# bjack205/LQR.jl

Hardware: NVIDIA B200
Metric: batched LQR KKT solves/sec (FP64) (higher is better)
Workload: dtype f64

## Files before the change

lqr.jl_b200/csrc/api.cu:

```cuda
#include <cstdio>
#include <cstring>

#include "common.cuh"

int32_t lqrb_fail(lqrb_context *h, int32_t code, const std::string &msg) {
    if (h) h->err = msg;
    return code;
}

int32_t lqrb_cuda_fail(lqrb_context *h, cudaError_t e, const char *what) {
    if (h) h->err = std::string(what) + ": " + cudaGetErrorString(e);
    return 1000 + (int32_t)e;
}

void *lqrb_scratch(lqrb_context *h, int slot, size_t bytes, int lane) {
    if (bytes == 0) bytes = 16;
    void *&cur = h->scratch[slot][lane];
    size_t &have = h->scratch_bytes[slot][lane];
    if (have >= bytes) return cur;
    if (cur) {
        cudaDeviceSynchronize();
        cudaFree(cur);
        cur = nullptr;
        have = 0;
    }
    void *p = nullptr;
    cudaError_t e = cudaMalloc(&p, bytes);
    if (e != cudaSuccess) {
        lqrb_cuda_fail(h, e, "cudaMalloc(scratch)");
        return nullptr;
    }
    cur = p;
    have = bytes;
    return p;
}

void *lqrb_pinned(lqrb_context *h, int lane, size_t bytes) {
    if (bytes == 0) bytes = 16;
    if (h->pinned_bytes[lane] >= bytes) return h->pinned[lane];
    if (h->pinned[lane]) {
        cudaStreamSynchronize(h->stream);
        cudaFreeHost(h->pinned[lane]);
        h->pinned[lane] = nullptr;
        h->pinned_bytes[lane] = 0;
    }
    void *p = nullptr;
    cudaError_t e = cudaMallocHost(&p, bytes);
    if (e != cudaSuccess) {
        lqrb_cuda_fail(h, e, "cudaMallocHost");
        return nullptr;
    }
    h->pinned[lane] = p;
    h->pinned_bytes[lane] = bytes;
    return p;
}

extern "C" int32_t lqrb_version(void) { return LQRB_VERSION; }

extern "C" int32_t lqrb_device_count(int32_t *count) {
    if (!count) return -1;
    int c = 0;
    cudaError_t e = cudaGetDeviceCount(&c);
    if (e != cudaSuccess) {
        cudaGetLastError();
        *count = 0;
        return 1000 + (int32_t)e;
    }
    *count = c;
    return 0;
}

extern "C" int32_t lqrb_create(lqrb_handle_t *handle, int32_t device) {
    if (!handle) return -1;
    *handle = nullptr;
    int c = 0;
    cudaError_t e = cudaGetDeviceCount(&c);
    if (e != cudaSuccess) {
        cudaGetLastError();
        return 1000 + (int32_t)e;
    }
    if (device < 0 || device >= c) return -2;
    lqrb_context *h = new lqrb_context();
    h->device = device;
    if ((e = cudaSetDevice(device)) != cudaSuccess) {
        delete h;
        return 1000 + (int32_t)e;
    }
    cudaDeviceProp prop;
    if ((e = cudaGetDeviceProperties(&prop, device)) != cudaSuccess) {
        delete h;
        return 1000 + (int32_t)e;
    }
    if (prop.major != 10) {
        delete h;
        return -2;
    }
    h->sm_count = prop.multiProcessorCount;
    cudaStreamCreateWithFlags(&h->own_stream, cudaStreamNonBlocking);
    cudaStreamCreateWithFlags(&h->copy_stream[0], cudaStreamNonBlocking);
    cudaStreamCreateWithFlags(&h->copy_stream[1], cudaStreamNonBlocking);
    for (auto &ev : h->ev) cudaEventCreateWithFlags(&ev, cudaEventDisableTiming);
    h->stream = h->own_stream;
    *handle = h;
    return 0;
}

extern "C" int32_t lqrb_destroy(lqrb_handle_t h) {
    if (!h) return -1;
    cudaSetDevice(h->device);
    cudaDeviceSynchronize();
    for (auto &slot : h->scratch)
        for (void *p : slot)
            if (p) cudaFree(p);
    for (void *p : h->pinned)
        if (p) cudaFreeHost(p);
    for (auto &kv : h->maps)
        if (kv.second.dev) cudaFree((void *)kv.second.dev);
    for (auto &kv : h->blobs)
        if (kv.second) cudaFree(kv.second);
    for (auto &ev : h->ev)
        if (ev) cudaEventDestroy(ev);
    cudaStreamDestroy(h->own_stream);
    cudaStreamDestroy(h->copy_stream[0]);
    cudaStreamDestroy(h->copy_stream[1]);
    delete h;
    return 0;
}

extern "C" const char *lqrb_last_error_string(lqrb_handle_t h) {
    return h ? h->err.c_str() : "null handle";
}

extern "C" int32_t lqrb_set_stream(lqrb_handle_t h, void *s) {
    if (!h) return -1;
    h->stream = s ? (cudaStream_t)s : h->own_stream;
    return 0;
}

extern "C" int32_t lqrb_synchronize(lqrb_handle_t h) {
    if (!h) return -1;
    LQRB_CUDA(h, cudaSetDevice(h->device));
    LQRB_CUDA(h, cudaStreamSynchronize(h->stream));
    return 0;
}

extern "C" int64_t lqrb_launch_count(lqrb_handle_t h) { return h ? h->launches : -1; }

extern "C" const char *lqrb_last_kernel_name(lqrb_handle_t h) {
    return h ? h->kernel_name.c_str() : "";
}

extern "C" int32_t lqrb_set_option(lqrb_handle_t h, const char *name, int64_t value) {
    if (!h) return -1;
    if (!name) return -2;
    h->options[name] = value;
    return 0;
}

extern "C" int64_t lqrb_padded_batch(int64_t batch) { return round_up(batch, LQRB_TILE); }

extern "C" int64_t lqrb_num_vars(int32_t n, int32_t m, int32_t N) {
    return (int64_t)N * n + (int64_t)(N - 1) * m;
}

extern "C" int64_t lqrb_num_cons(int32_t n, int32_t N, const int32_t *p) {
    int64_t P = (int64_t)(N - 1) * n;
    if (p)
        for (int k = 0; k < N; ++k) P += p[k];
    return P;
}

extern "C" int32_t lqrb_riccati_layout(int32_t n, int32_t m, int32_t N, int32_t flags,
                                       lqrb_riccati_layout_t *out) {
    if (n < 1) return -1;
    if (m < 1) return -2;
    if (N < 2) return -3;
    if (!out) return -5;
    out->rows_per_knot = lqrb_riccati_knot_rows(n, m);
    out->knot_count = (flags & LQRB_FLAG_LTI) ? 1 : N - 1;
    out->term_rows = tri(n) + 2 * n;
// ... 174 lines not shown
```

lqr.jl_b200/csrc/common.cuh:

```cuda
#pragma once
#include <cuda_runtime.h>
#include <stdint.h>

#include <algorithm>
#include <functional>
#include <map>
#include <string>
#include <vector>

#include "../../include/lqrb200.h"

#define LQRB_TILE 32

__host__ __device__ __forceinline__ int64_t packed_index(int64_t rows, int tile_w, int64_t row,
                                                         int64_t inst) {
    return ((inst / tile_w) * rows + row) * tile_w + (inst % tile_w);
}

__host__ __device__ constexpr int tri(int k) { return k * (k + 1) / 2; }
__host__ __device__ constexpr int tri_idx(int i, int j) { return j * (j + 1) / 2 + i; }
__host__ __device__ constexpr int sym_idx(int i, int j) { return i <= j ? tri_idx(i, j) : tri_idx(j, i); }

__host__ __device__ constexpr int hess_rows(int n, int mk, int hess) {
    return hess == LQRB_HESS_DIAG ? n + mk : hess == LQRB_HESS_BLOCKDIAG ? tri(n) + tri(mk) : tri(n + mk);
}

enum ScratchSlot {
    SCR_GAINS = 0,
    SCR_FACT,
    SCR_STAGE_A,
    SCR_STAGE_B,
    SCR_PACK_IN,
    SCR_PACK_IN2,
    SCR_PACK_OUT,
    SCR_PACK_OUT2,
    SCR_PACK_OUT3,
    SCR_MISC,
    SCR_SQP0,
    SCR_SQP1,
    SCR_SQP2,
    SCR_SQP3,
    SCR_KEEP_DATA,
    SCR_KEEP_REC,
    SCR_REFINE,
    SCR_REFINE_LIST,
    SCR_RICCATI_PAD,
    SCR_COUNT
};

struct Lane {
    cudaStream_t stream;
    int index;
};

struct RowMap;
struct DevMap {
    const RowMap *dev = nullptr;
    int64_t rows = 0;
};

struct lqrb_context {
    int device = 0;
    int sm_count = 148;
    cudaStream_t stream = nullptr;
    cudaStream_t own_stream = nullptr;
    cudaStream_t copy_stream[2] = {nullptr, nullptr};
    cudaEvent_t ev[8] = {};
    std::string err;
    std::string kernel_name;
    int64_t launches = 0;
    void *scratch[SCR_COUNT][2] = {};
    size_t scratch_bytes[SCR_COUNT][2] = {};
    void *pinned[2] = {};
    size_t pinned_bytes[2] = {};
    std::map<std::string, int64_t> options;
    std::map<std::string, struct DevMap> maps;
    std::map<std::string, void *> blobs;
    std::vector<int32_t> last_cond;
    int64_t last_refined = 0;
    std::string kept_key;
    int64_t kept_batch = 0;

    int64_t opt(const char *name, int64_t dflt) const {
        auto it = options.find(name);
        return it == options.end() ? dflt : it->second;
    }
};

int32_t lqrb_fail(lqrb_context *h, int32_t code, const std::string &msg);
int32_t lqrb_cuda_fail(lqrb_context *h, cudaError_t e, const char *what);
void *lqrb_scratch(lqrb_context *h, int slot, size_t bytes, int lane = 0);
void *lqrb_pinned(lqrb_context *h, int lane, size_t bytes);

struct HostArray {
    const void *ptr;
    int64_t bytes;
};
using ChunkBody = std::function<int32_t(Lane lane, int64_t cb, const void *const *in, void *const *out)>;
int32_t lqrb_for_chunks(lqrb_context *h, int64_t batch, int64_t chunk, const std::vector<HostArray> &inputs,
                        const std::vector<HostArray> &outputs, const ChunkBody &body);

#define LQRB_CUDA(h, call)                                              \
    do {                                                                \
        cudaError_t e__ = (call);                                       \
        if (e__ != cudaSuccess) return lqrb_cuda_fail((h), e__, #call); \
    } while (0)

#define LQRB_LAUNCH_CHECK(h, name)                                                    \
    do {                                                                              \
        (h)->launches++;                                                              \
        cudaError_t e__ = cudaGetLastError();                                         \
        if (e__ != cudaSuccess) return lqrb_cuda_fail((h), e__, "launch of " name);   \
    } while (0)

static inline int64_t round_up(int64_t a, int64_t b) { return (a + b - 1) / b * b; }

__host__ __device__ constexpr int lqrb_riccati_knot_rows(int n, int m) {
    const int f = n * n + n * m + n * (n + 1) / 2 + m * (m + 1) / 2 + n + m;
    return ((n == 8 || n == 12) && m <= 4) ? ((f + 1) & ~1) : f;
}

struct RowMap {
    int32_t array;
    int32_t offset;
    double fill;
};
#define LQRB_MAX_ARRAYS 16
struct ArrayTable {
    const double *ptr[LQRB_MAX_ARRAYS];
    int64_t stride[LQRB_MAX_ARRAYS];
};
struct ArrayTableOut {
    double *ptr[LQRB_MAX_ARRAYS];
    int64_t stride[LQRB_MAX_ARRAYS];
};

DevMap lqrb_get_map(lqrb_context *h, const std::string &key, std::vector<RowMap> (*build)(const int *),
                    const int *args);
DevMap lqrb_get_map(lqrb_context *h, const std::string &key, const std::vector<RowMap> &map);
DevMap lqrb_identity_map(lqrb_context *h, int64_t rows);
int32_t lqrb_gather_pack(lqrb_context *h, const DevMap &map, const ArrayTable &src, int64_t batch,
                         int tile_w, double *packed, cudaStream_t s);
int32_t lqrb_scatter_unpack(lqrb_context *h, const DevMap &map, const ArrayTableOut &dst,
                            int64_t batch, int tile_w, const double *packed, cudaStream_t s);

int lqrb_riccati_tile(const lqrb_context *h, int n, int m);
// ... 7 lines not shown
```

lqr.jl_b200/csrc/riccati.cu:

```cuda
#include <algorithm>
#include <cstdio>

#include "riccati_kernels.cuh"
#include "riccati_dmma_kernels.cuh"
#include "riccati_cta_kernels.cuh"

#define RICCATI_SIZES(X)                                                                                              \
    X(Tpi, 2, 1) X(Tpi, 3, 2) X(Tpi, 4, 1) X(Tpi, 4, 2) X(Tpi, 6, 3) X(Tpi, 2, 2) X(Tpi, 3, 1) X(Tpi, 3, 3)           \
    X(Tpi, 4, 3) X(Tpi, 5, 1) X(Tpi, 5, 2) X(Tpi, 5, 3) X(Tpi, 6, 1) X(Tpi, 6, 2)                                     \
    X(Dmma, 8, 1) X(Dmma, 8, 2) X(Dmma, 8, 3) X(Dmma, 8, 4) X(Dmma, 12, 1) X(Dmma, 12, 2) X(Dmma, 12, 3)              \
    X(Dmma, 12, 4)                                                                                                    \
    X(Cta, 16, 8) X(Cta, 16, 16) X(Cta, 24, 8) X(Cta, 24, 16) X(Cta, 32, 8) X(Cta, 32, 16) X(Cta, 48, 16) X(Cta, 64, 16)

namespace {
enum class RiccatiFamily { Tpi, Dmma, Cta, Pad, Coop };
struct RiccatiRoute {
    RiccatiFamily family;
    int n2 = 0, m2 = 0;
};
}

static RiccatiRoute riccati_route(const lqrb_context *h, int n, int m, bool data_aligned) {
    if (h->opt("riccati_variant", 0) == 2) return {RiccatiFamily::Coop};
    RiccatiFamily own = RiccatiFamily::Coop;
#define X(F_, N_, M_) \
    if (n == N_ && m == M_) own = RiccatiFamily::F_;
    RICCATI_SIZES(X)
#undef X
    if (own == RiccatiFamily::Tpi || (data_aligned && own != RiccatiFamily::Coop)) return {own};
    if (data_aligned && h->opt("riccati_pad", 1) != 0) {
#define X(F_, N_, M_) \
    if (RiccatiFamily::F_ != RiccatiFamily::Tpi && n <= N_ && m <= M_) return {RiccatiFamily::Pad, N_, M_};
        RICCATI_SIZES(X)
#undef X
    }
    return {RiccatiFamily::Coop};
}

int lqrb_riccati_tile(const lqrb_context *h, int n, int m) {
    return riccati_route(h, n, m, true).family == RiccatiFamily::Tpi ? LQRB_TILE : 1;
}

static std::vector<RowMap> riccati_knot_map(int n, int m, int N, int flags) {
    const int Kn = (flags & LQRB_FLAG_LTI) ? 1 : N - 1;
    std::vector<RowMap> map;
    map.reserve((size_t)Kn * (n * n + n * m + tri(n) + tri(m) + n + m));
    for (int k = 0; k < Kn; ++k) {
        for (int e = 0; e < n * n; ++e) map.push_back({0, k * n * n + e, 0.0});
        for (int e = 0; e < n * m; ++e) map.push_back({1, k * n * m + e, 0.0});
        for (int j = 0; j < n; ++j)
            for (int i = 0; i <= j; ++i) map.push_back({2, k * n * n + i + j * n, 0.0});
        for (int j = 0; j < m; ++j)
            for (int i = 0; i <= j; ++i) map.push_back({3, k * m * m + i + j * m, 0.0});
        for (int e = 0; e < n; ++e) map.push_back({4, k * n + e, 0.0});
        for (int e = 0; e < m; ++e) map.push_back({5, k * m + e, 0.0});
        if (lqrb_riccati_knot_rows(n, m) > n * n + n * m + tri(n) + tri(m) + n + m) map.push_back({-1, 0, 0.0});
    }
    return map;
}

static std::vector<RowMap> riccati_term_map(int n) {
    std::vector<RowMap> map;
    for (int j = 0; j < n; ++j)
        for (int i = 0; i <= j; ++i) map.push_back({6, i + j * n, 0.0});
    for (int e = 0; e < n; ++e) map.push_back({7, e, 0.0});
    for (int e = 0; e < n; ++e) map.push_back({8, e, 0.0});
    return map;
}

static std::vector<RowMap> riccati_gain_map(int n, int m, int N) {
    std::vector<RowMap> map;
    for (int k = 0; k < N - 1; ++k) {
        for (int e = 0; e < m * n; ++e) map.push_back({0, k * m * n + e, 0.0});
        for (int e = 0; e < m; ++e) map.push_back({1, k * m + e, 0.0});
    }
    return map;
}

static std::string key(const char *tag, int a, int b, int c, int d) {
    char buf[96];
    snprintf(buf, sizeof buf, "%s:%d:%d:%d:%d", tag, a, b, c, d);
    return buf;
}

static int32_t check_dims(lqrb_context *h, int n, int m, int N, int64_t batch) {
    if (!h) return -1;
    if (n < 1 || n > 128) return lqrb_fail(h, -2, "n out of range [1,128]");
    if (m < 1 || m > n) return lqrb_fail(h, -3, "m out of range [1,n]");
    if (N < 2) return lqrb_fail(h, -4, "N must be >= 2");
    if (batch < 0) return lqrb_fail(h, -5, "batch must be >= 0");
    return 0;
}

template <int n, int m>
static int32_t launch_tpi(lqrb_context *h, int N, int64_t batch, int lti, const double *knots,
                          const double *term, double *Z, double *gains, int32_t *info,
                          cudaStream_t s) {
    constexpr bool SMALL = (n * n + n * m) <= 20;
    constexpr int THREADS = SMALL ? 64 : 128, MINB = SMALL ? 8 : 1;
    const unsigned grid = (unsigned)((batch + THREADS - 1) / THREADS);
    if (lti) riccati_tpi_kernel<n, m, true, THREADS, MINB><<<grid, THREADS, 0, s>>>(knots, term, Z, gains, info, N, batch);
    else riccati_tpi_kernel<n, m, false, THREADS, MINB><<<grid, THREADS, 0, s>>>(knots, term, Z, gains, info, N, batch);
    char nm[64];
    snprintf(nm, sizeof nm, "riccati_tpi<%d,%d>%s%s", n, m, lti ? "[lti]" : "", SMALL ? "[64x8]" : "[128x1]");
    h->kernel_name = nm;
    LQRB_LAUNCH_CHECK(h, "riccati_tpi_kernel");
    return 0;
}

static int32_t launch_coop(lqrb_context *h, int n, int m, int N, int64_t batch, int lti,
                           const double *knots, const double *term, double *Z, double *gains,
                           int32_t *info, cudaStream_t s) {
    const size_t per = riccati_coop_smem_doubles(n, m) * sizeof(double);
    char nm[64];
    if (n + m <= 24) {
        constexpr int G = 32, THREADS = 128;
        const size_t smem = per * (THREADS / G);
        auto kern = riccati_coop_kernel<G, THREADS>;
        LQRB_CUDA(h, cudaFuncSetAttribute(kern, cudaFuncAttributeMaxDynamicSharedMemorySize, (int)smem));
        const unsigned grid = (unsigned)((batch + THREADS / G - 1) / (THREADS / G));
        kern<<<grid, THREADS, smem, s>>>(knots, term, Z, gains, info, n, m, N, lti, batch);
        snprintf(nm, sizeof nm, "riccati_coop<G=32>(n=%d,m=%d)", n, m);
    } else {
        constexpr int G = 256, THREADS = 256;
        if (per > 227 * 1024) return lqrb_fail(h, -2, "n,m too large for the shared-memory Riccati kernel");
        auto kern = riccati_coop_kernel<G, THREADS>;
        LQRB_CUDA(h, cudaFuncSetAttribute(kern, cudaFuncAttributeMaxDynamicSharedMemorySize, (int)per));
        kern<<<(unsigned)batch, THREADS, per, s>>>(knots, term, Z, gains, info, n, m, N, lti, batch);
        snprintf(nm, sizeof nm, "riccati_coop<G=256>(n=%d,m=%d)", n, m);
    }
    h->kernel_name = nm;
    LQRB_LAUNCH_CHECK(h, "riccati_coop_kernel");
    return 0;
}

template <int n, int m>
static int32_t launch_dmma(lqrb_context *h, int N, int64_t batch, int lti, const double *knots,
                           const double *term, double *Z, double *gains, int32_t *info,
                           cudaStream_t s) {
    constexpr int STAGES = 3, WARPS = 4, MINB = m == 1 ? 6 : 5;
    const size_t smem = rdmma::riccati_dmma_warp_smem(rdmma::Map<n, m>::F, STAGES) * WARPS;
    auto kern = rdmma::riccati_dmma_kernel<n, m, STAGES, WARPS, MINB>;
    LQRB_CUDA(h, cudaFuncSetAttribute(kern, cudaFuncAttributeMaxDynamicSharedMemorySize, (int)smem));
    const unsigned grid = (unsigned)((batch + WARPS - 1) / WARPS);
    kern<<<grid, WARPS * 32, smem, s>>>(knots, term, Z, gains, info, N, lti, batch);
    char nm[64];
    snprintf(nm, sizeof nm, "riccati_dmma<%d,%d>%s", n, m, lti ? "[lti]" : "");
    h->kernel_name = nm;
    LQRB_LAUNCH_CHECK(h, "riccati_dmma_kernel");
    return 0;
}

template <int n, int m>
static int32_t launch_cta(lqrb_context *h, int N, int64_t batch, int lti, const double *knots,
                          const double *term, double *Z, double *gains, int32_t *info, cudaStream_t s) {
    using C = rcta::Cfg<n, m>;
    auto kern = rcta::riccati_cta_kernel<n, m>;
    LQRB_CUDA(h, cudaFuncSetAttribute(kern, cudaFuncAttributeMaxDynamicSharedMemorySize, (int)C::SMEM));
    kern<<<(unsigned)batch, C::THREADS, C::SMEM, s>>>(knots, term, Z, gains, info, N, lti, batch);
    char nm[64];
    snprintf(nm, sizeof nm, "riccati_cta_dmma<%d,%d>%s", n, m, lti ? "[lti]" : "");
    h->kernel_name = nm;
    LQRB_LAUNCH_CHECK(h, "riccati_cta_kernel");
    return 0;
}

template <RiccatiFamily F, int n, int m>
static int32_t launch_sized(lqrb_context *h, int N, int64_t batch, int lti, const double *knots, const double *term,
                            double *Z, double *gains, int32_t *info, cudaStream_t s) {
    if constexpr (F == RiccatiFamily::Tpi) return launch_tpi<n, m>(h, N, batch, lti, knots, term, Z, gains, info, s);
    else if constexpr (F == RiccatiFamily::Dmma) return launch_dmma<n, m>(h, N, batch, lti, knots, term, Z, gains, info, s);
    else return launch_cta<n, m>(h, N, batch, lti, knots, term, Z, gains, info, s);
}

static int32_t launch_tuned(lqrb_context *h, RiccatiFamily family, int n, int m, int N, int64_t batch, int lti,
                            const double *knots, const double *term, double *Z, double *gains, int32_t *info,
                            cudaStream_t s) {
#define X(F_, N_, M_)                                                     \
    if (family == RiccatiFamily::F_ && n == N_ && m == M_)                \
        return launch_sized<RiccatiFamily::F_, N_, M_>(h, N, batch, lti, knots, term, Z, gains, info, s);
    RICCATI_SIZES(X)
#undef X
    return lqrb_fail(h, 1, "no tuned Riccati kernel for this size");
}


namespace {
struct RiccatiPadMaps {
    std::vector<RowMap> knots, term, z, gains;
};
}

static RiccatiPadMaps riccati_pad_maps(int n, int m, int N, int Kn, int n2, int m2) {
    RiccatiPadMaps M;
    const int F = lqrb_riccati_knot_rows(n, m), F2 = lqrb_riccati_knot_rows(n2, m2);
    const int nn = n * n, nm = n * m, tn = tri(n), tm = tri(m);
    for (int k = 0; k < Kn; ++k) {
        const int32_t b = k * F;
        const size_t start = M.knots.size();
        for (int j = 0; j < n2; ++j)
            for (int i = 0; i < n2; ++i) M.knots.push_back((i < n && j < n) ? RowMap{0, b + i + j * n, 0.0} : RowMap{-1, 0, 0.0});
        for (int j = 0; j < m2; ++j)
            for (int i = 0; i < n2; ++i)
                M.knots.push_back((i < n && j < m) ? RowMap{0, b + nn + i + j * n, 0.0} : RowMap{-1, 0, 0.0});
        for (int j = 0; j < n2; ++j)
            for (int i = 0; i <= j; ++i)
                M.knots.push_back(j < n ? RowMap{0, b + nn + nm + j * (j + 1) / 2 + i, 0.0} : RowMap{-1, 0, i == j ? 1.0 : 0.0});
        for (int j = 0; j < m2; ++j)
            for (int i = 0; i <= j; ++i)
                M.knots.push_back(j < m ? RowMap{0, b + nn + nm + tn + j * (j + 1) / 2 + i, 0.0} : RowMap{-1, 0, i == j ? 1.0 : 0.0});
        for (int i = 0; i < n2; ++i) M.knots.push_back(i < n ? RowMap{0, b + nn + nm + tn + tm + i, 0.0} : RowMap{-1, 0, 0.0});
        for (int i = 0; i < m2; ++i) M.knots.push_back(i < m ? RowMap{0, b + nn + nm + tn + tm + n + i, 0.0} : RowMap{-1, 0, 0.0});
        while (M.knots.size() - start < (size_t)F2) M.knots.push_back(RowMap{-1, 0, 0.0});
    }
    for (int j = 0; j < n2; ++j)
        for (int i = 0; i <= j; ++i) M.term.push_back(j < n ? RowMap{0, j * (j + 1) / 2 + i, 0.0} : RowMap{-1, 0, i == j ? 1.0 : 0.0});
    for (int i = 0; i < n2; ++i) M.term.push_back(i < n ? RowMap{0, tn + i, 0.0} : RowMap{-1, 0, 0.0});
    for (int i = 0; i < n2; ++i) M.term.push_back(i < n ? RowMap{0, tn + n + i, 0.0} : RowMap{-1, 0, 0.0});
    for (int k = 0; k < N; ++k) {
        for (int i = 0; i < n2; ++i) M.z.push_back(i < n ? RowMap{0, k * (n + m) + i, 0.0} : RowMap{-1, 0, 0.0});
        if (k < N - 1)
            for (int i = 0; i < m2; ++i) M.z.push_back(i < m ? RowMap{0, k * (n + m) + n + i, 0.0} : RowMap{-1, 0, 0.0});
    }
    const int GR = m * n + m;
    for (int k = 0; k < N - 1; ++k) {
        for (int j = 0; j < n2; ++j)
            for (int c = 0; c < m2; ++c) M.gains.push_back((c < m && j < n) ? RowMap{0, k * GR + c + m * j, 0.0} : RowMap{-1, 0, 0.0});
        for (int c = 0; c < m2; ++c) M.gains.push_back(c < m ? RowMap{0, k * GR + m * n + c, 0.0} : RowMap{-1, 0, 0.0});
    }
    return M;
}

static int32_t riccati_solve_padded(lqrb_context *h, int n, int m, int N, int n2, int m2, int64_t batch, int flags,
                                    const double *knots, const double *term, double *Z, double *gains, int32_t *info,
                                    Lane lane) {
    const RiccatiFamily family = riccati_route(h, n2, m2, true).family;
    if (family != RiccatiFamily::Dmma && family != RiccatiFamily::Cta)
        return lqrb_fail(h, 1, "padded Riccati size has no tensor-core kernel");
    const int lti = (flags & LQRB_FLAG_LTI) ? 1 : 0;
    const int Kn = lti ? 1 : N - 1;
    const int64_t F = lqrb_riccati_knot_rows(n, m), F2 = lqrb_riccati_knot_rows(n2, m2);
    const int64_t TR = tri(n) + 2 * n, TR2 = tri(n2) + 2 * n2;
    const int64_t ZR = (int64_t)N * n + (int64_t)(N - 1) * m, ZR2 = (int64_t)N * n2 + (int64_t)(N - 1) * m2;
    const int64_t GR = (int64_t)(N - 1) * (m * n + m), GR2 = (int64_t)(N - 1) * (m2 * n2 + m2);
    const std::string k0 = key("rpad", n, m, N, Kn) + key("->", n2, m2, 0, 0);
    DevMap mk, mt, mz, mg;
    if (h->maps.find(k0 + ":g") == h->maps.end()) {
        const RiccatiPadMaps M = riccati_pad_maps(n, m, N, Kn, n2, m2);
        mk = lqrb_get_map(h, k0 + ":k", M.knots);
        mt = lqrb_get_map(h, k0 + ":t", M.term);
        mz = lqrb_get_map(h, k0 + ":z", M.z);
        mg = lqrb_get_map(h, k0 + ":g", M.gains);
    } else {
        mk = h->maps[k0 + ":k"];
        mt = h->maps[k0 + ":t"];
        mz = h->maps[k0 + ":z"];
        mg = h->maps[k0 + ":g"];
    }
    if (mk.rows != Kn * F2 || mt.rows != TR2 || mz.rows != ZR2 || mg.rows != GR2) return lqrb_fail(h, 1, "pad map size mismatch");
    const int64_t per = Kn * F2 + TR2 + ZR2 + GR2;
    int64_t chunk = std::max<int64_t>(LQRB_TILE, ((int64_t)2 << 30) / (per * 8) / LQRB_TILE * LQRB_TILE);
    chunk = std::min(chunk, lqrb_padded_batch(batch));
    const size_t slice = ((size_t)chunk * per * 8 + 255) / 256 * 256;
    char *base = (char *)lqrb_scratch(h, SCR_RICCATI_PAD, slice, lane.index);
    if (!base) return 1000 + (int)cudaErrorMemoryAllocation;
    double *knots2 = (double *)base, *term2 = knots2 + chunk * Kn * F2, *Z2 = term2 + chunk * TR2, *gains2 = Z2 + chunk * ZR2;
    std::string name;
    for (int64_t first = 0; first < batch; first += chunk) {
        const int64_t cb = std::min(chunk, batch - first);
        ArrayTable src = {};
        src.ptr[0] = knots + first * Kn * F;
        src.stride[0] = Kn * F;
        int32_t rc = lqrb_gather_pack(h, mk, src, cb, 1, knots2, lane.stream);
        if (rc) return rc;
        src.ptr[0] = term + first * TR;
        src.stride[0] = TR;
        rc = lqrb_gather_pack(h, mt, src, cb, 1, term2, lane.stream);
        if (rc) return rc;
        rc = launch_tuned(h, family, n2, m2, N, cb, lti, knots2, term2, Z2, gains2, info ? info + first : nullptr,
                          lane.stream);
        if (rc) return rc;
        name = h->kernel_name;
        ArrayTableOut o = {};
        o.ptr[0] = Z + first * ZR;
        o.stride[0] = ZR;
        rc = lqrb_scatter_unpack(h, mz, o, cb, 1, Z2, lane.stream);
        if (rc) return rc;
        o.ptr[0] = gains + first * GR;
        o.stride[0] = GR;
        rc = lqrb_scatter_unpack(h, mg, o, cb, 1, gains2, lane.stream);
        if (rc) return rc;
    }
    char nm[64];
    snprintf(nm, sizeof nm, " <- (%d,%d) padded", n, m);
    h->kernel_name = name + nm;
    return 0;
}

static int32_t riccati_solve_on(lqrb_context *h, int n, int m, int N, int64_t batch, int flags,
                                const double *knots, const double *term, double *Z, double *gains,
                                int32_t *info, Lane lane) {
    if (batch == 0) return 0;
    const RiccatiRoute r = riccati_route(h, n, m, ((uintptr_t)knots & 15) == 0);
    const int lti = (flags & LQRB_FLAG_LTI) ? 1 : 0;
    switch (r.family) {
    case RiccatiFamily::Pad:
        return riccati_solve_padded(h, n, m, N, r.n2, r.m2, batch, flags, knots, term, Z, gains, info, lane);
    case RiccatiFamily::Tpi:
    case RiccatiFamily::Dmma:
    case RiccatiFamily::Cta:
        return launch_tuned(h, r.family, n, m, N, batch, lti, knots, term, Z, gains, info, lane.stream);
    case RiccatiFamily::Coop:
        break;
    }
    return launch_coop(h, n, m, N, batch, lti, knots, term, Z, gains, info, lane.stream);
}

extern "C" int32_t lqrb_riccati_solve_packed_f64(lqrb_handle_t h, int32_t n, int32_t m, int32_t N,
                                                 int64_t batch, int32_t flags, const double *knots,
                                                 const double *term, double *Z, double *gains,
                                                 int32_t *info) {
    int32_t rc = check_dims(h, n, m, N, batch);
    if (rc) return rc;
    if (!knots) return lqrb_fail(h, -7, "knots is NULL");
    if (!term) return lqrb_fail(h, -8, "term is NULL");
    if (!Z) return lqrb_fail(h, -9, "Z is NULL");
    LQRB_CUDA(h, cudaSetDevice(h->device));
    if (!gains) {
        const size_t bytes = (size_t)lqrb_padded_batch(batch) * (N - 1) * (m * n + m) * sizeof(double);
        gains = (double *)lqrb_scratch(h, SCR_GAINS, bytes);
        if (!gains) return 1000 + (int)cudaErrorMemoryAllocation;
    }
    return riccati_solve_on(h, n, m, N, batch, flags, knots, term, Z, gains, info, Lane{h->stream, 0});
}

static int32_t riccati_pack_on(lqrb_context *h, int n, int m, int N, int64_t batch, int flags,
                               const double *A, const double *B, const double *Q, const double *R,
                               const double *q, const double *r, const double *Qf, const double *qf,
                               const double *x0, double *knots, double *term, cudaStream_t s) {
    const int Kn = (flags & LQRB_FLAG_LTI) ? 1 : N - 1;
    const int tile = lqrb_riccati_tile(h, n, m);
    ArrayTable t = {};
    const double *ptrs[9] = {A, B, Q, R, q, r, Qf, qf, x0};
    const int64_t strides[9] = {(int64_t)Kn * n * n, (int64_t)Kn * n * m, (int64_t)Kn * n * n,
                                (int64_t)Kn * m * m, (int64_t)Kn * n,     (int64_t)Kn * m,
                                (int64_t)n * n,      n,                   n};
    for (int i = 0; i < 9; ++i) {
        t.ptr[i] = ptrs[i];
        t.stride[i] = strides[i];
    }
    DevMap km = lqrb_get_map(h, key("rk", n, m, N, flags & LQRB_FLAG_LTI), riccati_knot_map(n, m, N, flags));
    DevMap tm = lqrb_get_map(h, key("rt", n, 0, 0, 0), riccati_term_map(n));
    int32_t rc = lqrb_gather_pack(h, km, t, batch, tile, knots, s);
    if (rc) return rc;
    return lqrb_gather_pack(h, tm, t, batch, tile, term, s);
}

extern "C" int32_t lqrb_riccati_pack_f64(lqrb_handle_t h, int32_t n, int32_t m, int32_t N,
                                         int64_t batch, int32_t flags, const double *A,
                                         const double *B, const double *Q, const double *R,
                                         const double *q, const double *r, const double *Qf,
                                         const double *qf, const double *x0, double *knots,
                                         double *term) {
    int32_t rc = check_dims(h, n, m, N, batch);
    if (rc) return rc;
    if (!A) return lqrb_fail(h, -7, "A is NULL");
    if (!B) return lqrb_fail(h, -8, "B is NULL");
    if (!Q) return lqrb_fail(h, -9, "Q is NULL");
    if (!R) return lqrb_fail(h, -10, "R is NULL");
    if (!Qf) return lqrb_fail(h, -13, "Qf is NULL");
    if (!x0) return lqrb_fail(h, -15, "x0 is NULL");
    if (!knots) return lqrb_fail(h, -16, "knots is NULL");
    if (!term) return lqrb_fail(h, -17, "term is NULL");
    LQRB_CUDA(h, cudaSetDevice(h->device));
    return riccati_pack_on(h, n, m, N, batch, flags, A, B, Q, R, q, r, Qf, qf, x0, knots, term, h->stream);
}

static int32_t riccati_unpack_on(lqrb_context *h, int n, int m, int N, int64_t batch,
                                 const double *Zp, const double *gains, double *Z, double *K,
                                 double *kff, cudaStream_t s) {
    const int tile = lqrb_riccati_tile(h, n, m);
    const int64_t NN = lqrb_num_vars(n, m, N);
    ArrayTableOut t = {};
    t.ptr[0] = Z;
    t.stride[0] = NN;
    int32_t rc = lqrb_scatter_unpack(h, lqrb_identity_map(h, NN), t, batch, tile, Zp, s);
    if (rc) return rc;
    if (K || kff) {
// ... 161 lines not shown
```

lqr.jl_b200/csrc/riccati_kernels.cuh:

```cuda
#pragma once
#include "smallmat.cuh"

template <int n, int m>
struct RiccatiRows {
    static constexpr int oA = 0, oB = n * n, oQ = oB + n * m, oR = oQ + tri(n), oq = oR + tri(m),
                         orr = oq + n, F = lqrb_riccati_knot_rows(n, m);
    static constexpr int TR = tri(n) + 2 * n;
    static constexpr int GR = m * n + m;
    static constexpr int W = n + m;
};

template <int n, int m>
__device__ __forceinline__ int riccati_step(const double *A, const double *B, const double *Q,
                                            const double *R, const double *q, const double *r,
                                            double *P, double *p, double *K, double *kff) {
    double PB[n * m], PA[n * n], E[tri(m)], Einv[m], Kraw[m * n], rr[m];
    SM_UNROLL
    for (int j = 0; j < m; ++j)
        SM_UNROLL
        for (int i = 0; i < n; ++i) {
            double s = 0.0;
            SM_UNROLL
            for (int l = 0; l < n; ++l) s = fma(P[sym_idx(i, l)], B[l + j * n], s);
            PB[i + j * n] = s;
        }
    SM_UNROLL
    for (int j = 0; j < n; ++j)
        SM_UNROLL
        for (int i = 0; i < n; ++i) {
            double s = 0.0;
            SM_UNROLL
            for (int l = 0; l < n; ++l) s = fma(P[sym_idx(i, l)], A[l + j * n], s);
            PA[i + j * n] = s;
        }
    SM_UNROLL
    for (int j = 0; j < m; ++j)
        SM_UNROLL
        for (int i = 0; i <= j; ++i) {
            double s = R[tri_idx(i, j)];
            SM_UNROLL
            for (int l = 0; l < n; ++l) s = fma(B[l + i * n], PB[l + j * n], s);
            E[tri_idx(i, j)] = s;
        }
    SM_UNROLL
    for (int j = 0; j < n; ++j)
        SM_UNROLL
        for (int i = 0; i < m; ++i) {
            double s = 0.0;
            SM_UNROLL
            for (int l = 0; l < n; ++l) s = fma(B[l + i * n], PA[l + j * n], s);
            Kraw[i + j * m] = s;
            K[i + j * m] = s;
        }
    SM_UNROLL
    for (int i = 0; i < m; ++i) {
        double s = r[i];
        SM_UNROLL
        for (int l = 0; l < n; ++l) s = fma(B[l + i * n], p[l], s);
        rr[i] = s;
        kff[i] = s;
    }
    const int st = chol_packed<m>(E, Einv);
    SM_UNROLL
    for (int j = 0; j < n; ++j) solve_chol<m>(E, Einv, K + j * m);
    solve_chol<m>(E, Einv, kff);
    double pn[n];
    SM_UNROLL
    for (int i = 0; i < n; ++i) {
        double s = q[i];
        SM_UNROLL
        for (int l = 0; l < n; ++l) s = fma(A[l + i * n], p[l], s);
        SM_UNROLL
        for (int l = 0; l < m; ++l) s = fma(-K[l + i * m], rr[l], s);
        pn[i] = s;
    }
    SM_UNROLL
    for (int j = 0; j < n; ++j)
        SM_UNROLL
        for (int i = 0; i <= j; ++i) {
            double s = Q[tri_idx(i, j)];
            SM_UNROLL
            for (int l = 0; l < n; ++l) s = fma(A[l + i * n], PA[l + j * n], s);
            SM_UNROLL
            for (int l = 0; l < m; ++l) s = fma(-Kraw[l + i * m], K[l + j * m], s);
            P[tri_idx(i, j)] = s;
        }
    SM_UNROLL
    for (int i = 0; i < n; ++i) p[i] = pn[i];
    return st;
}

template <int n, int m, bool LTI, int THREADS, int MINB>
__global__ void __launch_bounds__(THREADS, MINB)
    riccati_tpi_kernel(const double *__restrict__ knots, const double *__restrict__ term,
                       double *__restrict__ Z, double *__restrict__ gains,
                       int32_t *__restrict__ info, int N, int64_t batch) {
    using L = RiccatiRows<n, m>;
    const int64_t inst = (int64_t)blockIdx.x * THREADS + threadIdx.x;
    if (inst >= batch) return;
    const int64_t tile = inst >> 5;
    const int lane = (int)(inst & 31);
    const int Kn = LTI ? 1 : N - 1;
    const double *kb = knots + tile * Kn * L::F * 32 + lane;
    const double *tb = term + tile * L::TR * 32 + lane;
    double *zb = Z + tile * ((int64_t)N * n + (int64_t)(N - 1) * m) * 32 + lane;
    double *gb = gains + tile * (int64_t)(N - 1) * L::GR * 32 + lane;

    double P[tri(n)], p[n];
    SM_UNROLL
    for (int e = 0; e < tri(n); ++e) P[e] = ld_stream(tb + e * 32);
    SM_UNROLL
    for (int e = 0; e < n; ++e) p[e] = ld_stream(tb + (tri(n) + e) * 32);

    double A[n * n], B[n * m];
    int st_all = 0;
    for (int k = N - 2; k >= 0; --k) {
        const double *kp = kb + (int64_t)(LTI ? 0 : k) * L::F * 32;
        double Q[tri(n)], R[tri(m)], q[n], r[m];
        SM_UNROLL
        for (int e = 0; e < n * n; ++e) A[e] = ld_keep(kp + (L::oA + e) * 32);
        SM_UNROLL
        for (int e = 0; e < n * m; ++e) B[e] = ld_keep(kp + (L::oB + e) * 32);
        SM_UNROLL
        for (int e = 0; e < tri(n); ++e) Q[e] = ld_stream(kp + (L::oQ + e) * 32);
        SM_UNROLL
        for (int e = 0; e < tri(m); ++e) R[e] = ld_stream(kp + (L::oR + e) * 32);
        SM_UNROLL
        for (int e = 0; e < n; ++e) q[e] = ld_stream(kp + (L::oq + e) * 32);
        SM_UNROLL
        for (int e = 0; e < m; ++e) r[e] = ld_stream(kp + (L::orr + e) * 32);
        double K[m * n], kff[m];
        const int st = riccati_step<n, m>(A, B, Q, R, q, r, P, p, K, kff);
        if (st != 0 && st_all == 0) st_all = (k + 1) * 1000 + st;
        double *gk = gb + (int64_t)k * L::GR * 32;
        SM_UNROLL
        for (int e = 0; e < m * n; ++e) gk[e * 32] = K[e];
        SM_UNROLL
        for (int e = 0; e < m; ++e) gk[(m * n + e) * 32] = kff[e];
    }
    if (info) info[inst] = st_all;

    double x[n];
    SM_UNROLL
    for (int e = 0; e < n; ++e) x[e] = ld_stream(tb + (tri(n) + n + e) * 32);
    for (int k = 0; k < N - 1; ++k) {
        const double *kp = kb + (int64_t)(LTI ? 0 : k) * L::F * 32;
        const double *gk = gb + (int64_t)k * L::GR * 32;
        double K[m * n], kff[m], u[m], xn[n];
        SM_UNROLL
        for (int e = 0; e < n * n; ++e) A[e] = ld_stream(kp + (L::oA + e) * 32);
        SM_UNROLL
        for (int e = 0; e < n * m; ++e) B[e] = ld_stream(kp + (L::oB + e) * 32);
        SM_UNROLL
        for (int e = 0; e < m * n; ++e) K[e] = gk[e * 32];
        SM_UNROLL
        for (int e = 0; e < m; ++e) kff[e] = gk[(m * n + e) * 32];
        double *zk = zb + (int64_t)k * L::W * 32;
        SM_UNROLL
        for (int i = 0; i < n; ++i) __stcs(zk + i * 32, x[i]);
        SM_UNROLL
        for (int i = 0; i < m; ++i) {
            double s = -kff[i];
            SM_UNROLL
            for (int l = 0; l < n; ++l) s = fma(-K[i + l * m], x[l], s);
            u[i] = s;
            __stcs(zk + (n + i) * 32, s);
        }
        SM_UNROLL
        for (int i = 0; i < n; ++i) {
            double s = 0.0;
            SM_UNROLL
            for (int l = 0; l < n; ++l) s = fma(A[i + l * n], x[l], s);
            SM_UNROLL
            for (int l = 0; l < m; ++l) s = fma(B[i + l * n], u[l], s);
            xn[i] = s;
        }
        SM_UNROLL
        for (int i = 0; i < n; ++i) x[i] = xn[i];
    }
    double *zN = zb + (int64_t)(N - 1) * L::W * 32;
    SM_UNROLL
    for (int i = 0; i < n; ++i) __stcs(zN + i * 32, x[i]);
}

template <int G>
__device__ __forceinline__ void group_sync() {
    if (G <= 32)
        __syncwarp();
    else
        __syncthreads();
}

__host__ __device__ inline size_t riccati_coop_smem_doubles(int n, int m) {
    return (size_t)4 * n * n + 4 * n * m + m * m + 4 * n + 3 * m + 8;
}

template <int G, int THREADS>
__global__ void __launch_bounds__(THREADS)
    riccati_coop_kernel(const double *__restrict__ knots, const double *__restrict__ term,
                        double *__restrict__ Z, double *__restrict__ gains,
                        int32_t *__restrict__ info, int n, int m, int N, int lti, int64_t batch) {
    extern __shared__ double smem[];
    constexpr int IPC = THREADS / G;
    const int g = threadIdx.x / G, t = threadIdx.x % G;
    const int64_t inst_raw = (int64_t)blockIdx.x * IPC + g;
    const bool active = inst_raw < batch;
    const int64_t inst = active ? inst_raw : batch - 1;
    const int nn = n * n, nm = n * m, tn = tri(n), tm = tri(m);
    const int F = lqrb_riccati_knot_rows(n, m), TR = tn + 2 * n, GR = m * n + m, W = n + m;
    const int Kn = lti ? 1 : N - 1;
    double *s = smem + (size_t)g * riccati_coop_smem_doubles(n, m);
    double *P = s, *Pn = P + nn, *PA = Pn + nn, *A = PA + nn, *B = A + nn, *PB = B + nm,
           *Kraw = PB + nm, *K = Kraw + nm, *E = K + nm, *p = E + m * m, *pn = p + n, *x = pn + n,
           *xn = x + n, *rr = xn + n, *kff = rr + m, *u = kff + m;
    const double *rec = knots + inst * (int64_t)Kn * F;
    const double *tb = term + inst * TR;
    double *zb = Z + inst * ((int64_t)N * n + (int64_t)(N - 1) * m);
    double *gb = gains + inst * (int64_t)(N - 1) * GR;
    int st_all = 0;

    for (int e = t; e < nn; e += G) {
        const int i = e % n, j = e / n;
        P[e] = tb[sym_idx(i, j)];
    }
    for (int e = t; e < n; e += G) p[e] = tb[tn + e];
    group_sync<G>();

    for (int k = N - 2; k >= 0; --k) {
        const double *kp = rec + (int64_t)(lti ? 0 : k) * F;
        const double *Qp = kp + nn + nm, *Rp = Qp + tn, *qp = Rp + tm, *rp = qp + n;
        for (int e = t; e < nn; e += G) A[e] = kp[e];
        for (int e = t; e < nm; e += G) B[e] = kp[nn + e];
        group_sync<G>();
        for (int e = t; e < nn + nm; e += G) {
            const bool isA = e < nn;
            const int ee = isA ? e : e - nn;
            const int i = ee % n, j = ee / n;
            const double *col = (isA ? A : B) + j * n;
            double acc = 0.0;
// ... 116 lines not shown
```

Before: 116.7 million.

## Pin late-knot dynamics and gains in L2 with evict_last hints across passes

In the time-varying Riccati kernel, the A/B loads and the K/kff gain stores for the first W knots, which the forward pass reads first, now use an L2 evict_last cache policy. W is sized from a fraction of the device L2 capacity divided by the per-knot footprint across the batch. After the forward pass uses a knot, its lines are demoted back to evict_normal with applypriority. The goal is to turn the forward pass's DRAM reads of A, B and the gains into L2 hits, at the cost of extra applypriority instructions and possible L2 contention with other traffic.

```diff
diff --git a/lqr.jl_b200/csrc/api.cu b/lqr.jl_b200/csrc/api.cu
--- a/lqr.jl_b200/csrc/api.cu
+++ b/lqr.jl_b200/csrc/api.cu
@@ -96,6 +96,7 @@
         return -2;
     }
     h->sm_count = prop.multiProcessorCount;
+    h->l2_bytes = prop.l2CacheSize;
     cudaStreamCreateWithFlags(&h->own_stream, cudaStreamNonBlocking);
     cudaStreamCreateWithFlags(&h->copy_stream[0], cudaStreamNonBlocking);
     cudaStreamCreateWithFlags(&h->copy_stream[1], cudaStreamNonBlocking);
diff --git a/lqr.jl_b200/csrc/common.cuh b/lqr.jl_b200/csrc/common.cuh
--- a/lqr.jl_b200/csrc/common.cuh
+++ b/lqr.jl_b200/csrc/common.cuh
@@ -62,6 +62,7 @@
 struct lqrb_context {
     int device = 0;
     int sm_count = 148;
+    int64_t l2_bytes = 126 << 20;
     cudaStream_t stream = nullptr;
     cudaStream_t own_stream = nullptr;
     cudaStream_t copy_stream[2] = {nullptr, nullptr};
diff --git a/lqr.jl_b200/csrc/riccati.cu b/lqr.jl_b200/csrc/riccati.cu
--- a/lqr.jl_b200/csrc/riccati.cu
+++ b/lqr.jl_b200/csrc/riccati.cu
@@ -92,6 +92,11 @@
     return 0;
 }
 
+#ifndef RTPI_SHARE
+#define RTPI_SHARE 0.5
+#endif
+constexpr double RTPI_L2_SHARE = RTPI_SHARE;
+
 template <int n, int m>
 static int32_t launch_tpi(lqrb_context *h, int N, int64_t batch, int lti, const double *knots,
                           const double *term, double *Z, double *gains, int32_t *info,
@@ -99,8 +104,10 @@
     constexpr bool SMALL = (n * n + n * m) <= 20;
     constexpr int THREADS = SMALL ? 64 : 128, MINB = SMALL ? 8 : 1;
     const unsigned grid = (unsigned)((batch + THREADS - 1) / THREADS);
-    if (lti) riccati_tpi_kernel<n, m, true, THREADS, MINB><<<grid, THREADS, 0, s>>>(knots, term, Z, gains, info, N, batch);
-    else riccati_tpi_kernel<n, m, false, THREADS, MINB><<<grid, THREADS, 0, s>>>(knots, term, Z, gains, info, N, batch);
+    const int64_t kept_per_knot = lqrb_padded_batch(batch) * (n * n + n * m + m * n + m) * 8;
+    const int W = (int)std::min<int64_t>(N - 1, (int64_t)(RTPI_L2_SHARE * h->l2_bytes) / kept_per_knot);
+    if (lti) riccati_tpi_kernel<n, m, true, THREADS, MINB><<<grid, THREADS, 0, s>>>(knots, term, Z, gains, info, N, batch, 0);
+    else riccati_tpi_kernel<n, m, false, THREADS, MINB><<<grid, THREADS, 0, s>>>(knots, term, Z, gains, info, N, batch, W);
     char nm[64];
     snprintf(nm, sizeof nm, "riccati_tpi<%d,%d>%s%s", n, m, lti ? "[lti]" : "", SMALL ? "[64x8]" : "[128x1]");
     h->kernel_name = nm;
diff --git a/lqr.jl_b200/csrc/riccati_kernels.cuh b/lqr.jl_b200/csrc/riccati_kernels.cuh
--- a/lqr.jl_b200/csrc/riccati_kernels.cuh
+++ b/lqr.jl_b200/csrc/riccati_kernels.cuh
@@ -90,11 +90,27 @@
     return st;
 }
 
+__device__ __forceinline__ double ld_keep_last(const double *p, uint64_t pol) {
+    double v;
+    asm volatile("ld.global.nc.L2::cache_hint.f64 %0, [%1], %2;" : "=d"(v) : "l"(p), "l"(pol));
+    return v;
+}
+__device__ __forceinline__ void st_keep_last(double *p, double v, uint64_t pol) {
+    asm volatile("st.global.L2::cache_hint.f64 [%0], %1, %2;" ::"l"(p), "d"(v), "l"(pol) : "memory");
+}
+__device__ __forceinline__ void l2_normal_span(const double *p, int bytes, int lane) {
+    const uintptr_t end = reinterpret_cast<uintptr_t>(p) + bytes;
+    for (uintptr_t a = (reinterpret_cast<uintptr_t>(p) & ~(uintptr_t)127) + lane * 128; a < end; a += 32 * 128)
+        asm volatile("applypriority.global.L2::evict_normal [%0], 128;" ::"l"(a) : "memory");
+}
+
 template <int n, int m, bool LTI, int THREADS, int MINB>
 __global__ void __launch_bounds__(THREADS, MINB)
     riccati_tpi_kernel(const double *__restrict__ knots, const double *__restrict__ term,
                        double *__restrict__ Z, double *__restrict__ gains,
-                       int32_t *__restrict__ info, int N, int64_t batch) {
+                       int32_t *__restrict__ info, int N, int64_t batch, int W) {
+    uint64_t keep;
+    asm("createpolicy.fractional.L2::evict_last.b64 %0, 1.0;" : "=l"(keep));
     using L = RiccatiRows<n, m>;
     const int64_t inst = (int64_t)blockIdx.x * THREADS + threadIdx.x;
     if (inst >= batch) return;
@@ -117,10 +133,17 @@
     for (int k = N - 2; k >= 0; --k) {
         const double *kp = kb + (int64_t)(LTI ? 0 : k) * L::F * 32;
         double Q[tri(n)], R[tri(m)], q[n], r[m];
-        SM_UNROLL
-        for (int e = 0; e < n * n; ++e) A[e] = ld_keep(kp + (L::oA + e) * 32);
-        SM_UNROLL
-        for (int e = 0; e < n * m; ++e) B[e] = ld_keep(kp + (L::oB + e) * 32);
+        if (!LTI && k < W) {
+            SM_UNROLL
+            for (int e = 0; e < n * n; ++e) A[e] = ld_keep_last(kp + (L::oA + e) * 32, keep);
+            SM_UNROLL
+            for (int e = 0; e < n * m; ++e) B[e] = ld_keep_last(kp + (L::oB + e) * 32, keep);
+        } else {
+            SM_UNROLL
+            for (int e = 0; e < n * n; ++e) A[e] = ld_keep(kp + (L::oA + e) * 32);
+            SM_UNROLL
+            for (int e = 0; e < n * m; ++e) B[e] = ld_keep(kp + (L::oB + e) * 32);
+        }
         SM_UNROLL
         for (int e = 0; e < tri(n); ++e) Q[e] = ld_stream(kp + (L::oQ + e) * 32);
         SM_UNROLL
@@ -133,10 +156,17 @@
         const int st = riccati_step<n, m>(A, B, Q, R, q, r, P, p, K, kff);
         if (st != 0 && st_all == 0) st_all = (k + 1) * 1000 + st;
         double *gk = gb + (int64_t)k * L::GR * 32;
-        SM_UNROLL
-        for (int e = 0; e < m * n; ++e) gk[e * 32] = K[e];
-        SM_UNROLL
-        for (int e = 0; e < m; ++e) gk[(m * n + e) * 32] = kff[e];
+        if (!LTI && k < W) {
+            SM_UNROLL
+            for (int e = 0; e < m * n; ++e) st_keep_last(gk + e * 32, K[e], keep);
+            SM_UNROLL
+            for (int e = 0; e < m; ++e) st_keep_last(gk + (m * n + e) * 32, kff[e], keep);
+        } else {
+            SM_UNROLL
+            for (int e = 0; e < m * n; ++e) gk[e * 32] = K[e];
+            SM_UNROLL
+            for (int e = 0; e < m; ++e) gk[(m * n + e) * 32] = kff[e];
+        }
     }
     if (info) info[inst] = st_all;
 
@@ -155,6 +185,10 @@
         for (int e = 0; e < m * n; ++e) K[e] = gk[e * 32];
         SM_UNROLL
         for (int e = 0; e < m; ++e) kff[e] = gk[(m * n + e) * 32];
+        if (!LTI && k < W) {
+            l2_normal_span(kp - lane, L::oQ * 32 * 8, lane);
+            l2_normal_span(gk - lane, L::GR * 32 * 8, lane);
+        }
         double *zk = zb + (int64_t)k * L::W * 32;
         SM_UNROLL
         for (int i = 0; i < n; ++i) __stcs(zk + i * 32, x[i]);
```

Result: no change. 117.2 million (median of 6 runs) (+0.4%).

## Add quad-thread TMA-pipelined Riccati kernel for n=4,m=1 large batches

Applied to the files above, without the earlier changes.

Adds a specialized kernel for the n=4, m=1 time-varying case that splits each instance across 4 threads (one per state column), so more threads work on each solve. It is a persistent kernel that streams knot data through a 7-stage bulk-async-copy/mbarrier pipeline with L2 evict hints, keeping A/B resident for the forward pass. Gains are kept in shared memory for the forward rollout. This adds shuffle traffic and a block-wide sync per knot, and applies only to aligned, non-LTI inputs with batch at least 8192 and at most 128 knots.

```diff
diff --git a/lqr.jl_b200/csrc/riccati.cu b/lqr.jl_b200/csrc/riccati.cu
--- a/lqr.jl_b200/csrc/riccati.cu
+++ b/lqr.jl_b200/csrc/riccati.cu
@@ -4,6 +4,7 @@
 #include "riccati_kernels.cuh"
 #include "riccati_dmma_kernels.cuh"
 #include "riccati_cta_kernels.cuh"
+#include "riccati_quad_kernels.cuh"
 
 #define RICCATI_SIZES(X)                                                                                              \
     X(Tpi, 2, 1) X(Tpi, 3, 2) X(Tpi, 4, 1) X(Tpi, 4, 2) X(Tpi, 6, 3) X(Tpi, 2, 2) X(Tpi, 3, 1) X(Tpi, 3, 3)           \
@@ -13,15 +14,20 @@
     X(Cta, 16, 8) X(Cta, 16, 16) X(Cta, 24, 8) X(Cta, 24, 16) X(Cta, 32, 8) X(Cta, 32, 16) X(Cta, 48, 16) X(Cta, 64, 16)
 
 namespace {
-enum class RiccatiFamily { Tpi, Dmma, Cta, Pad, Coop };
+enum class RiccatiFamily { Tpi, Quad, Dmma, Cta, Pad, Coop };
 struct RiccatiRoute {
     RiccatiFamily family;
     int n2 = 0, m2 = 0;
 };
 }
 
-static RiccatiRoute riccati_route(const lqrb_context *h, int n, int m, bool data_aligned) {
+#define RICCATI_QUAD_MIN_BATCH 8192
+
+static RiccatiRoute riccati_route(const lqrb_context *h, int n, int m, bool data_aligned, int N, int64_t batch,
+                                  bool lti) {
     if (h->opt("riccati_variant", 0) == 2) return {RiccatiFamily::Coop};
+    if (n == 4 && m == 1 && data_aligned && !lti && N - 1 <= rquad::MAX_KNOTS && batch >= RICCATI_QUAD_MIN_BATCH)
+        return {RiccatiFamily::Quad};
     RiccatiFamily own = RiccatiFamily::Coop;
 #define X(F_, N_, M_) \
     if (n == N_ && m == M_) own = RiccatiFamily::F_;
@@ -38,7 +44,7 @@
 }
 
 int lqrb_riccati_tile(const lqrb_context *h, int n, int m) {
-    return riccati_route(h, n, m, true).family == RiccatiFamily::Tpi ? LQRB_TILE : 1;
+    return riccati_route(h, n, m, true, 2, 0, false).family == RiccatiFamily::Tpi ? LQRB_TILE : 1;
 }
 
 static std::vector<RowMap> riccati_knot_map(int n, int m, int N, int flags) {
@@ -131,6 +137,17 @@
     }
     h->kernel_name = nm;
     LQRB_LAUNCH_CHECK(h, "riccati_coop_kernel");
+    return 0;
+}
+
+static int32_t launch_quad(lqrb_context *h, int N, int64_t batch, const double *knots, const double *term, double *Z,
+                           double *gains, int32_t *info, cudaStream_t s) {
+    const size_t smem = rquad::smem_bytes(N);
+    LQRB_CUDA(h, cudaFuncSetAttribute(rquad::riccati_quad_kernel, cudaFuncAttributeMaxDynamicSharedMemorySize, (int)smem));
+    const unsigned grid = (unsigned)std::min<int64_t>((batch + LQRB_TILE - 1) / LQRB_TILE, h->sm_count);
+    rquad::riccati_quad_kernel<<<grid, rquad::THREADS, smem, s>>>(knots, term, Z, gains, info, N, batch);
+    h->kernel_name = "riccati_quad<4,1>";
+    LQRB_LAUNCH_CHECK(h, "riccati_quad_kernel");
     return 0;
 }
 
@@ -234,7 +251,7 @@
 static int32_t riccati_solve_padded(lqrb_context *h, int n, int m, int N, int n2, int m2, int64_t batch, int flags,
                                     const double *knots, const double *term, double *Z, double *gains, int32_t *info,
                                     Lane lane) {
-    const RiccatiFamily family = riccati_route(h, n2, m2, true).family;
+    const RiccatiFamily family = riccati_route(h, n2, m2, true, N, 0, flags & LQRB_FLAG_LTI).family;
     if (family != RiccatiFamily::Dmma && family != RiccatiFamily::Cta)
         return lqrb_fail(h, 1, "padded Riccati size has no tensor-core kernel");
     const int lti = (flags & LQRB_FLAG_LTI) ? 1 : 0;
@@ -301,9 +318,11 @@
                                 const double *knots, const double *term, double *Z, double *gains,
                                 int32_t *info, Lane lane) {
     if (batch == 0) return 0;
-    const RiccatiRoute r = riccati_route(h, n, m, ((uintptr_t)knots & 15) == 0);
     const int lti = (flags & LQRB_FLAG_LTI) ? 1 : 0;
+    const RiccatiRoute r = riccati_route(h, n, m, ((uintptr_t)knots & 15) == 0, N, batch, lti);
     switch (r.family) {
+    case RiccatiFamily::Quad:
+        return launch_quad(h, N, batch, knots, term, Z, gains, info, lane.stream);
     case RiccatiFamily::Pad:
         return riccati_solve_padded(h, n, m, N, r.n2, r.m2, batch, flags, knots, term, Z, gains, info, lane);
     case RiccatiFamily::Tpi:
diff --git a/lqr.jl_b200/csrc/riccati_quad_kernels.cuh b/lqr.jl_b200/csrc/riccati_quad_kernels.cuh
--- /dev/null
+++ b/lqr.jl_b200/csrc/riccati_quad_kernels.cuh
@@ -0,0 +1,216 @@
+#pragma once
+#include "riccati_dmma_kernels.cuh"
+#include "riccati_kernels.cuh"
+
+namespace rquad {
+
+constexpr int n = 4, m = 1;
+using L = RiccatiRows<n, m>;
+constexpr int THREADS = 128;
+constexpr int STAGES = 7;
+constexpr int MAX_KNOTS = 128;
+constexpr int AB = L::oQ;
+constexpr uint32_t REC_BYTES = L::F * 32 * 8;
+constexpr uint32_t AB_BYTES = AB * 32 * 8;
+
+__host__ __device__ inline size_t smem_bytes(int N) {
+    return (size_t)STAGES * REC_BYTES + (size_t)(N - 1) * L::GR * 32 * 8 + STAGES * 8;
+}
+static_assert(STAGES * REC_BYTES + MAX_KNOTS * L::GR * 32 * 8 + STAGES * 8 <= 227 * 1024, "shared memory");
+
+__device__ __forceinline__ uint64_t policy_evict_last() {
+    uint64_t p;
+    asm volatile("createpolicy.fractional.L2::evict_last.b64 %0, 1.0;" : "=l"(p));
+    return p;
+}
+__device__ __forceinline__ uint64_t policy_evict_first() {
+    uint64_t p;
+    asm volatile("createpolicy.fractional.L2::evict_first.b64 %0, 1.0;" : "=l"(p));
+    return p;
+}
+__device__ __forceinline__ void bulk_g2s_hint(void *dst, const void *src, uint32_t bytes, uint64_t *bar, uint64_t pol) {
+    asm volatile(
+        "cp.async.bulk.shared::cluster.global.mbarrier::complete_tx::bytes.L2::cache_hint [%0], [%1], %2, [%3], %4;" ::"r"(
+            rdmma::smem_u32(dst)),
+        "l"(src), "r"(bytes), "r"(rdmma::smem_u32(bar)), "l"(pol)
+        : "memory");
+}
+
+__device__ __forceinline__ void issue(int64_t g, const double *knots, double *stages, uint64_t *full, int N,
+                                      int64_t ntiles, uint64_t pol_keep, uint64_t pol_drop) {
+    const int J = 2 * (N - 1);
+    const int64_t tile = blockIdx.x + (g / J) * gridDim.x;
+    if (tile >= ntiles) return;
+    const int r = (int)(g % J);
+    const bool bwd = r < N - 1;
+    const int k = bwd ? N - 2 - r : r - (N - 1);
+    const double *src = knots + (tile * (N - 1) + k) * L::F * 32;
+    double *dst = stages + (g % STAGES) * (L::F * 32);
+    uint64_t *bar = full + g % STAGES;
+    if (bwd) {
+        rdmma::mbar_expect_tx(bar, REC_BYTES);
+        bulk_g2s_hint(dst, src, AB_BYTES, bar, pol_keep);
+        bulk_g2s_hint(dst + AB * 32, src + AB * 32, REC_BYTES - AB_BYTES, bar, pol_drop);
+    } else {
+        rdmma::mbar_expect_tx(bar, AB_BYTES);
+        bulk_g2s_hint(dst, src, AB_BYTES, bar, pol_drop);
+    }
+}
+
+__device__ __forceinline__ double pick(const double (&v)[n], int j) {
+    return j == 0 ? v[0] : j == 1 ? v[1] : j == 2 ? v[2] : v[3];
+}
+
+__global__ void __launch_bounds__(THREADS, 1)
+    riccati_quad_kernel(const double *__restrict__ knots, const double *__restrict__ term, double *__restrict__ Z,
+                        double *__restrict__ gains, int32_t *__restrict__ info, int N, int64_t batch) {
+    extern __shared__ __align__(16) double qsm[];
+    double *stages = qsm;
+    double *gs = stages + STAGES * (L::F * 32);
+    uint64_t *full = (uint64_t *)(gs + (size_t)(N - 1) * L::GR * 32);
+    const int tid = threadIdx.x, ii = tid >> 2, j = tid & 3;
+    const int64_t ntiles = (batch + 31) / 32;
+    uint64_t pol_keep = 0, pol_drop = 0;
+    if (tid == 0) {
+        pol_keep = policy_evict_last();
+        pol_drop = policy_evict_first();
+        for (int s = 0; s < STAGES; ++s) rdmma::mbar_init(full + s, 1);
+        asm volatile("fence.mbarrier_init.release.cluster;" ::: "memory");
+        for (int s = 0; s < STAGES; ++s) issue(s, knots, stages, full, N, ntiles, pol_keep, pol_drop);
+    }
+    __syncthreads();
+
+    int64_t g = 0;
+    auto wait = [&]() -> const double * {
+        rdmma::mbar_wait(full + g % STAGES, (uint32_t)((g / STAGES) & 1));
+        return stages + (g % STAGES) * (L::F * 32) + ii;
+    };
+    auto release = [&]() {
+        __syncthreads();
+        if (tid == 0) issue(g + STAGES, knots, stages, full, N, ntiles, pol_keep, pol_drop);
+        ++g;
+    };
+
+    for (int64_t tile = blockIdx.x; tile < ntiles; tile += gridDim.x) {
+        const int64_t inst = tile * 32 + ii;
+        const bool active = inst < batch;
+        const double *tb = term + tile * L::TR * 32 + ii;
+        double *zb = Z + tile * ((int64_t)N * n + (int64_t)(N - 1) * m) * 32 + ii;
+        double *gb = gains + tile * (int64_t)(N - 1) * L::GR * 32 + ii;
+        double *gsi = gs + ii;
+
+        double P[tri(n)], p[n];
+        SM_UNROLL
+        for (int e = 0; e < tri(n); ++e) P[e] = ld_stream(tb + e * 32);
+        SM_UNROLL
+        for (int e = 0; e < n; ++e) p[e] = ld_stream(tb + (tri(n) + e) * 32);
+
+        int st_all = 0;
+        for (int k = N - 2; k >= 0; --k) {
+            const double *s = wait();
+            double A[n * n], B[n], Aj[n], Qj[n];
+            SM_UNROLL
+            for (int e = 0; e < n * n; ++e) A[e] = s[(L::oA + e) * 32];
+            SM_UNROLL
+            for (int e = 0; e < n; ++e) B[e] = s[(L::oB + e) * 32];
+            SM_UNROLL
+            for (int l = 0; l < n; ++l) Aj[l] = s[(L::oA + l + j * n) * 32];
+            SM_UNROLL
+            for (int i = 0; i < n; ++i) Qj[i] = s[(L::oQ + sym_idx(i, j)) * 32];
+            const double R = s[L::oR * 32], qj = s[(L::oq + j) * 32], r = s[L::orr * 32];
+
+            double PB[n], PA[n];
+            SM_UNROLL
+            for (int i = 0; i < n; ++i) {
+                double t = 0.0;
+                SM_UNROLL
+                for (int l = 0; l < n; ++l) t = fma(P[sym_idx(i, l)], B[l], t);
+                PB[i] = t;
+            }
+            SM_UNROLL
+            for (int i = 0; i < n; ++i) {
+                double t = 0.0;
+                SM_UNROLL
+                for (int l = 0; l < n; ++l) t = fma(P[sym_idx(i, l)], Aj[l], t);
+                PA[i] = t;
+            }
+            double E[1] = {R};
+            SM_UNROLL
+            for (int l = 0; l < n; ++l) E[0] = fma(B[l], PB[l], E[0]);
+            double Kraw = 0.0;
+            SM_UNROLL
+            for (int l = 0; l < n; ++l) Kraw = fma(B[l], PA[l], Kraw);
+            double rr = r;
+            SM_UNROLL
+            for (int l = 0; l < n; ++l) rr = fma(B[l], p[l], rr);
+            double Kr[n];
+            SM_UNROLL
+            for (int i = 0; i < n; ++i) Kr[i] = __shfl_sync(0xffffffffu, Kraw, i, 4);
+            double Einv[1];
+            const int st = chol_packed<m>(E, Einv);
+            double K = Kraw, kff = rr;
+            solve_chol<m>(E, Einv, &K);
+            solve_chol<m>(E, Einv, &kff);
+            double pn = qj;
+            SM_UNROLL
+            for (int l = 0; l < n; ++l) pn = fma(Aj[l], p[l], pn);
+            pn = fma(-K, rr, pn);
+            double col[n];
+            SM_UNROLL
+            for (int i = 0; i < n; ++i) {
+                double t = Qj[i];
+                SM_UNROLL
+                for (int l = 0; l < n; ++l) t = fma(A[l + i * n], PA[l], t);
+                col[i] = fma(-Kr[i], K, t);
+            }
+            if (st != 0 && st_all == 0) st_all = (k + 1) * 1000 + st;
+            SM_UNROLL
+            for (int jj = 0; jj < n; ++jj)
+                SM_UNROLL
+                for (int i = 0; i <= jj; ++i) P[tri_idx(i, jj)] = __shfl_sync(0xffffffffu, col[i], jj, 4);
+            SM_UNROLL
+            for (int i = 0; i < n; ++i) p[i] = __shfl_sync(0xffffffffu, pn, i, 4);
+
+            double *gk = gsi + k * L::GR * 32;
+            gk[j * 32] = K;
+            if (j == 0) gk[n * 32] = kff;
+            if (active) {
+                double *gg = gb + (int64_t)k * L::GR * 32;
+                __stcs(gg + j * 32, K);
+                if (j == 0) __stcs(gg + n * 32, kff);
+            }
+            release();
+        }
+        if (info && active && j == 0) info[inst] = st_all;
+
+        double x[n];
+        SM_UNROLL
+        for (int e = 0; e < n; ++e) x[e] = ld_stream(tb + (tri(n) + n + e) * 32);
+        for (int k = 0; k < N - 1; ++k) {
+            const double *s = wait();
+            double Ar[n];
+            SM_UNROLL
+            for (int l = 0; l < n; ++l) Ar[l] = s[(L::oA + j + l * n) * 32];
+            const double Bj = s[(L::oB + j) * 32];
+            const double *gk = gsi + k * L::GR * 32;
+            double u = -gk[n * 32];
+            SM_UNROLL
+            for (int l = 0; l < n; ++l) u = fma(-gk[l * 32], x[l], u);
+            double xn = 0.0;
+            SM_UNROLL
+            for (int l = 0; l < n; ++l) xn = fma(Ar[l], x[l], xn);
+            xn = fma(Bj, u, xn);
+            if (active) {
+                double *zk = zb + (int64_t)k * L::W * 32;
+                __stcs(zk + j * 32, pick(x, j));
+                if (j == 0) __stcs(zk + n * 32, u);
+            }
+            SM_UNROLL
+            for (int i = 0; i < n; ++i) x[i] = __shfl_sync(0xffffffffu, xn, i, 4);
+            release();
+        }
+        if (active) __stcs(zb + (int64_t)(N - 1) * L::W * 32 + j * 32, pick(x, j));
+    }
+}
+
+}
```

Result: slower. 115.4 million before, 35.64 million after, median of 6 (-69.1%).
